# danikiyasseh/SAIS

Hardware: AMD Instinct MI355X
Metric: frames/sec ViT-S/16 fwd+bwd, 224x224 32-frame clips (higher is better)
Workload: dtype bf16; 1 GPU; BASELINE config 2: ViT-S/16 + 4-layer temporal encoder + SupCon prototype loss, fwd+bwd+SGD, 8 clips x 32 frames x 224x224 per GPU (global 8 clips), random-init weights, RGB stream; clips_per_gpu=8, frames_per_clip=32, streams=1, parallelism=dp1, launch=hipGraph replay, last_block_cls_only=True

## Files before the change

sais_amd/csrc/gemm.hip:

```cpp
#include "gemm_nt_tile.hpp"

namespace {

template <int EPI>
__global__ __launch_bounds__(256) void gemm_nt_kernel(NtParams p) {
    __shared__ __attribute__((aligned(16))) char smem[4 * TILE_BYTES];
    const int tid = threadIdx.x, lane = tid & 63;
    const int wid = __builtin_amdgcn_readfirstlane(tid >> 6);
    const int wr = wid >> 1, wc = wid & 1, g = lane >> 4, li = lane & 15;
    const int ntn = p.N / BN;
    const int tile = xcd_remap(blockIdx.x, gridDim.x);
    const int n0 = (tile % ntn) * BN, m0 = (tile / ntn) * BM;

    const int sub = lane >> 3, spos = lane & 7, schunk = spos ^ sub;
    const bf16* asrc[4]; const bf16* bsrc[4];
#pragma unroll
    for (int j = 0; j < 4; ++j) {
        const int r = 8 * (4 * wid + j) + sub;
        int m = m0 + r;
        m = m < p.M ? m : p.M - 1;
        asrc[j] = p.A + (size_t)m * p.lda + schunk * 8;
        bsrc[j] = p.B + (size_t)(n0 + perm_row(r)) * p.ldb + schunk * 8;
    }
    auto issue = [&](int stage, int k0) {
        char* s = smem + stage * 2 * TILE_BYTES + (4 * wid) * 1024;
#pragma unroll
        for (int j = 0; j < 4; ++j) {
            glds16(asrc[j] + k0, s + j * 1024);
            glds16(bsrc[j] + k0, s + TILE_BYTES + j * 1024);
        }
    };

    f32x4 acc[4][4];
#pragma unroll
    for (int i = 0; i < 4; ++i)
#pragma unroll
        for (int j = 0; j < 4; ++j) acc[i][j] = f32x4{0, 0, 0, 0};

    int nk = p.K / BK, kbase = 0;
    if constexpr (EPI == SAIS_EPI_RAW_SLABS_F32) {
        const int per = (nk + (int)gridDim.y - 1) / (int)gridDim.y;
        kbase = blockIdx.y * per;
        nk = min(per, nk - kbase);
        if (nk <= 0) nk = 0;
    }
    if (nk > 0) issue(0, kbase * BK);
    __syncthreads();
    float bias[16];
    EpiAux aux;
    for (int kt = 0; kt < nk; ++kt) {
        const int cur = kt & 1;
        if (kt + 1 < nk) issue(cur ^ 1, (kbase + kt + 1) * BK);
        const char* sa = smem + cur * 2 * TILE_BYTES;
        const char* sb = sa + TILE_BYTES;
        if constexpr (EPI != SAIS_EPI_RAW_SLABS_F32)
            if (kt == nk - 1) epilogue_loads<EPI>(p, m0 + wr * 64, li, n0 + wc * 64 + 16 * g, bias, aux);
#pragma unroll
        for (int ks = 0; ks < 2; ++ks) {
            bf16x8 fa[4], fb[4];
#pragma unroll
            for (int t = 0; t < 4; ++t) {
                fa[t] = *(const bf16x8*)(sa + swz(wr * 64 + t * 16 + li, ks * 4 + g));
                fb[t] = *(const bf16x8*)(sb + swz(wc * 64 + t * 16 + li, ks * 4 + g));
            }
#pragma unroll
            for (int mt = 0; mt < 4; ++mt)
#pragma unroll
                for (int nt = 0; nt < 4; ++nt) acc[mt][nt] = mfma16(fb[nt], fa[mt], acc[mt][nt]);
        }
        __syncthreads();
    }

#pragma unroll
    for (int mt = 0; mt < 4; ++mt) {
        int m = m0 + wr * 64 + mt * 16 + li;
        if (m >= p.M) continue;
        float v[16];
#pragma unroll
        for (int nt = 0; nt < 4; ++nt)
#pragma unroll
            for (int r = 0; r < 4; ++r) v[4 * nt + r] = acc[mt][nt][r];
        if constexpr (EPI == SAIS_EPI_RAW_SLABS_F32) {
            float* o = (float*)p.out + ((size_t)blockIdx.y * p.M + m) * p.ldo + n0 + wc * 64 + 16 * g;
#pragma unroll
            for (int i = 0; i < 4; ++i) *(f32x4*)(o + 4 * i) = f32x4{v[4 * i], v[4 * i + 1], v[4 * i + 2], v[4 * i + 3]};
        } else {
            epilogue<EPI>(p, m, n0 + wc * 64 + 16 * g, v, bias, aux, mt);
        }
    }
}

__global__ __launch_bounds__(256) void splitk_finish_kernel(const float* ws, int ks, int M, int N, int lds, const float* bias,
                                                            const float* rowscale, const float* aux, int ldaux, float* out32,
                                                            int ldo32, bf16* out16, int ldo16) {
    const int n4 = N >> 2;
    for (long i = blockIdx.x * 256L + threadIdx.x; i < (long)M * n4; i += (long)gridDim.x * 256) {
        const int m = (int)(i / n4), n = (int)(i - (long)m * n4) * 4;
        f32x4 y = *(const f32x4*)(ws + (size_t)m * lds + n);
        for (int z = 1; z < ks; ++z) y += *(const f32x4*)(ws + ((size_t)z * M + m) * lds + n);
        if (bias) y += *(const f32x4*)(bias + n);
        if (rowscale) y *= rowscale[m];
        if (aux) y += *(const f32x4*)(aux + (size_t)m * ldaux + n);
        if (out32) *(f32x4*)(out32 + (size_t)m * ldo32 + n) = y;
        if (out16) {
            bf16x4 o;
            o[0] = (bf16)y[0]; o[1] = (bf16)y[1]; o[2] = (bf16)y[2]; o[3] = (bf16)y[3];
            *(bf16x4*)(out16 + (size_t)m * ldo16 + n) = o;
        }
    }
}

#ifdef SAIS_NT_STAMP
__device__ unsigned long long g_nt_stamps[8][16];
#define NTSTAMP(i) do { if (blockIdx.x == 0 && titer == 2 && lane == 0) g_nt_stamps[wid][i] = __builtin_readcyclecounter(); } while (0)
#else
#define NTSTAMP(i) do { } while (0)
#endif
#ifndef SAIS_NT_ABL
#define SAIS_NT_ABL 0
#endif
template <int EPI>
__global__ __launch_bounds__(512, 2) void gemm_nt_w8p_kernel(NtParams p, int ntiles) {
    extern __shared__ __attribute__((aligned(16))) char smem[];
    CLK_STAMP(EPI == SAIS_EPI_BIAS_GELU_GRAD_BF16 ? 1 : EPI == SAIS_EPI_MUL_BF16 ? 2 : 0);
    [[maybe_unused]] const int abl_role = (SAIS_NT_ABL & 4) ? (blockIdx.x & 1) : (SAIS_NT_ABL & 8) ? ((blockIdx.x >> 8) & 1) : -1;
    const bool do_k = !(SAIS_NT_ABL & 1) && abl_role != 1, do_e = !(SAIS_NT_ABL & 2) && abl_role != 0;
    const int tid = threadIdx.x, lane = tid & 63;
    const int wid = __builtin_amdgcn_readfirstlane(tid >> 6);
    const int wr = wid >> 2, wc = wid & 3, g = lane >> 4, li = lane & 15;
    const int ntn = p.N / BN;
    const int sub = lane >> 3, spos = lane & 7, schunk = spos ^ sub;
    const bf16* asrc[2]; const bf16* bsrc[2];
    auto set_tile = [&](int v, int& m0, int& n0) {
        const int tile = xcd_remap(v, ntiles);
        n0 = (tile % ntn) * BN; m0 = (tile / ntn) * BM;
#pragma unroll
        for (int j = 0; j < 2; ++j) {
            const int r = 8 * (2 * wid + j) + sub;
            int m = m0 + r;
            m = m < p.M ? m : p.M - 1;
            asrc[j] = p.A + (size_t)m * p.lda + schunk * 8;
            bsrc[j] = p.B + (size_t)(n0 + perm_row32(r)) * p.ldb + schunk * 8;
        }
    };
    char* const sW = smem + 3 * TILE_BYTES;
    auto issue_a = [&](int kt) {
        char* s = smem + (kt % 3) * TILE_BYTES + (2 * wid) * 1024;
#pragma unroll
        for (int j = 0; j < 2; ++j) glds16(asrc[j] + kt * BK, s + j * 1024);
    };
    auto issue_w = [&](int kt) {
        char* s = sW + (kt & 1) * TILE_BYTES + (2 * wid) * 1024;
#pragma unroll
        for (int j = 0; j < 2; ++j) glds16(bsrc[j] + kt * BK, s + j * 1024);
    };
    const int nk = p.K / BK;
    constexpr int SROW = (EPI == SAIS_EPI_BIAS_F32) ? 2 : (EPI == SAIS_EPI_BIAS_RESID_F32) ? 2 : (EPI == SAIS_EPI_PATCH_F32) ? 2
                       : (EPI == SAIS_EPI_BIAS_GELU_GRAD_BF16 || EPI == SAIS_EPI_BIAS_GELU_GRADQ_BF16) ? 2 : 1;
    const int nstores = 4 * (SROW + ((EPI == SAIS_EPI_BIAS_RESID_F32 || EPI == SAIS_EPI_BIAS_GELU_BF16) && p.out2 ? 1 : 0));

    const bool do_pf = nk == 6 && ntn >= 8 && ntn <= 16 && wid == 0;
    unsigned pf_keep = 0;
    auto prefetch_a = [&](int pm0, int tcol) {
        const int per = (BM + ntn - 1) / ntn;
        const int row = tcol * per + (lane >> 2);
        if ((lane >> 2) < per && row < BM) {
            int m = pm0 + row;
            m = m < p.M ? m : p.M - 1;
            const bf16* q = p.A + (size_t)m * p.lda + (2 + (lane & 3)) * 64;
            asm volatile("global_load_dword %0, %1, off" : "=v"(pf_keep) : "v"(q) : "memory");
        }
    };
    int v = blockIdx.x, m0, n0;
    if (v >= ntiles) return;
    set_tile(v, m0, n0);
    if (do_k) {
        issue_a(0);
        issue_w(0);
        if (nk > 1) issue_a(1);
    }
    if (nk > 1) asm volatile("s_waitcnt vmcnt(2)" ::: "memory"); else asm volatile("s_waitcnt vmcnt(0)" ::: "memory");
    __builtin_amdgcn_s_barrier();
    [[maybe_unused]] int titer = -1;
    for (;;) {
        ++titer;
        NTSTAMP(0);
        f32x4 acc[4][2];
#pragma unroll
        for (int i = 0; i < 4; ++i)
#pragma unroll
            for (int j = 0; j < 2; ++j) acc[i][j] = f32x4{0, 0, 0, 0};
        float bias[8];
        EpiAux8 aux;
        __builtin_amdgcn_s_setprio(2);
        for (int kt = 0; kt < (do_k ? nk : 0); ++kt) {
            if (kt + 1 < nk) issue_w(kt + 1);
            if (kt + 2 < nk) issue_a(kt + 2);
            const char* sa = smem + (kt % 3) * TILE_BYTES;
            const char* sb = sW + (kt & 1) * TILE_BYTES;
            if (kt == nk - 1 && do_e) epilogue_loads8<EPI>(p, m0 + wr * 64, li, n0 + wc * 32 + 8 * g, bias, aux);
#pragma unroll
            for (int ks = 0; ks < 2; ++ks) {
                bf16x8 fa[4], fb[2];
#pragma unroll
                for (int t = 0; t < 4; ++t) fa[t] = *(const bf16x8*)(sa + swz(wr * 64 + t * 16 + li, ks * 4 + g));
#pragma unroll
                for (int t = 0; t < 2; ++t) fb[t] = *(const bf16x8*)(sb + swz(wc * 32 + t * 16 + li, ks * 4 + g));
#pragma unroll
                for (int mt = 0; mt < 4; ++mt)
#pragma unroll
                    for (int nt = 0; nt < 2; ++nt) acc[mt][nt] = mfma16(fb[nt], fa[mt], acc[mt][nt]);
            }
            if (kt + 2 < nk) asm volatile("s_waitcnt vmcnt(2) lgkmcnt(0)" ::: "memory");
            else if (kt + 1 < nk) asm volatile("s_waitcnt vmcnt(0) lgkmcnt(0)" ::: "memory");
            else asm volatile("s_waitcnt lgkmcnt(0)" ::: "memory");
            NTSTAMP(1 + 2 * kt);
            __builtin_amdgcn_s_barrier();
            NTSTAMP(2 + 2 * kt);
        }
        __builtin_amdgcn_s_setprio(0);
        const int cm0 = m0, cn0 = n0;
        const int nv = v + gridDim.x;
        const bool more = nv < ntiles;
        asm volatile("" ::"v"(pf_keep));
        if (more) {
            set_tile(nv, m0, n0);
            if (do_k) {
                issue_a(0);
                issue_w(0);
                if (nk > 1) issue_a(1);
                if (do_pf) prefetch_a(m0, xcd_remap(nv, ntiles) % ntn);
            }
        }
        if (SAIS_NT_ABL) {
            if (!do_k) epilogue_loads8<EPI>(p, cm0 + wr * 64, li, cn0 + wc * 32 + 8 * g, bias, aux);
            if (!do_e) {
#pragma unroll
                for (int mt = 0; mt < 4; ++mt)
#pragma unroll
                    for (int nt = 0; nt < 2; ++nt) asm volatile("" ::"v"(acc[mt][nt]));
            }
        }
#pragma unroll
        for (int mt = 0; mt < (do_e ? 4 : 0); ++mt) {
            const int m = cm0 + wr * 64 + mt * 16 + li;
            if (m >= p.M) continue;
            float vv[8];
#pragma unroll
            for (int nt = 0; nt < 2; ++nt)
#pragma unroll
                for (int r = 0; r < 4; ++r) vv[4 * nt + r] = acc[mt][nt][r];
            epilogue8<EPI>(p, m, cn0 + wc * 32 + 8 * g, vv, bias, aux, mt);
        }
        NTSTAMP(13);
        if (!more) break;
        v = nv;
        const int allow = (cm0 + BM <= p.M && nk > 1) ? nstores + 2 + (do_pf ? 1 : 0) : 0;
        if (allow == 6) asm volatile("s_waitcnt vmcnt(6)" ::: "memory");
        else if (allow == 7) asm volatile("s_waitcnt vmcnt(7)" ::: "memory");
        else if (allow == 10) asm volatile("s_waitcnt vmcnt(10)" ::: "memory");
        else if (allow == 11) asm volatile("s_waitcnt vmcnt(11)" ::: "memory");
        else if (allow == 14) asm volatile("s_waitcnt vmcnt(14)" ::: "memory");
        else if (allow == 15) asm volatile("s_waitcnt vmcnt(15)" ::: "memory");
        else asm volatile("s_waitcnt vmcnt(0)" ::: "memory");
        NTSTAMP(14);
        __builtin_amdgcn_s_barrier();
        NTSTAMP(15);
    }
}

#ifdef SAIS_NT_STAMP
extern "C" int sais_debug_nt_stamps(unsigned long long* host_out) {
    return hipMemcpyFromSymbol(host_out, HIP_SYMBOL(g_nt_stamps), sizeof(unsigned long long) * 8 * 16) == hipSuccess ? 0 : -2;
}
#endif

}

extern "C" int sais_gemm_nt_row_(const SaisGemm* g, void* stream);
extern "C" int sais_gemm_nt_exp_(const SaisGemm* g, int nt_grid, void* stream);
CLK_EXPORT(gemm)

template <int E>
static int launch_nt(const NtParams& p, dim3 grid, bool big, int nt_grid, hipStream_t stream) {
    if (big) {
        if (!sais_dyn_lds_once<gemm_nt_w8p_kernel<E>>(5 * TILE_BYTES)) return SAIS_ERR_LAUNCH;
        const int nt = (int)grid.x;
        hipLaunchKernelGGL(gemm_nt_w8p_kernel<E>, dim3(nt < nt_grid ? nt : nt_grid), dim3(512), 5 * TILE_BYTES, stream, p, nt);
    } else {
        hipLaunchKernelGGL(gemm_nt_kernel<E>, grid, dim3(256), 0, stream, p);
    }
    return sais_check_launch();
}
#define NT_CASE(E) case E: return launch_nt<E>(p, grid, big, nt_grid, (hipStream_t)stream);

extern "C" int sais_gemm_nt(const SaisGemm* g, void* stream) {
    SAIS_ENTER();
    if (!g || !g->A || !g->B || !g->out) return SAIS_ERR_ARG;
    if (g->M <= 0 || g->N % BN || g->K % BK || g->lda % 8 || g->ldb % 8 || g->ldo % 8) return SAIS_ERR_ARG;
    if ((g->epilogue == SAIS_EPI_BIAS_GELU_GRAD_BF16 || g->epilogue == SAIS_EPI_BIAS_GELU_GRADQ_BF16) && !g->out2) return SAIS_ERR_ARG;
    if (g->epilogue == SAIS_EPI_BIAS_GELU_GRADQ_BF16 && (g->ldo2 % 16 || ((uintptr_t)g->out2 & 15))) return SAIS_ERR_ARG;
    if (g->epilogue == SAIS_EPI_MULQ_BF16 && (!g->aux || g->ldaux % 16 || ((uintptr_t)g->aux & 15))) return SAIS_ERR_ARG;
    if ((g->epilogue == SAIS_EPI_MUL_BF16 || g->epilogue == SAIS_EPI_DGELU_BF16 || g->epilogue == SAIS_EPI_DRELU_BF16 ||
         g->epilogue == SAIS_EPI_BIAS_RESID_F32) && !g->aux)
        return SAIS_ERR_ARG;
    const NtParams p = nt_params(g);
    if (g->rowscale && g->epilogue != SAIS_EPI_BIAS_RESID_F32) return SAIS_ERR_ARG;
    const dim3 grid = nt_tiles(g);
    const bool big = g->M >= 8192;
    static const int nt_grid_env = sais_env_int("SAIS_NT_GRID", 0);
    const int nt_grid = nt_grid_env > 0 ? nt_grid_env : 512;
    if (g->epilogue == SAIS_EPI_RAW_SLABS_F32) {
        if (big || g->grp_in < 1 || g->grp_in > g->K / BK || g->ldo % 4) return SAIS_ERR_ARG;
        hipLaunchKernelGGL(gemm_nt_kernel<SAIS_EPI_RAW_SLABS_F32>, dim3(grid.x, g->grp_in), dim3(256), 0, (hipStream_t)stream, p);
        return sais_check_launch();
    }
    if (big && g->N == 384 && (g->epilogue == SAIS_EPI_BIAS_BF16 || (g->epilogue == SAIS_EPI_BIAS_RESID_F32 && !g->out2)))
        return sais_gemm_nt_row_(g, stream);
    if (big && g->rowscale) return SAIS_ERR_ARG;
#if SAIS_EXPERIMENTAL
    if (big)
        if (const int r = sais_gemm_nt_exp_(g, nt_grid, stream)) return r > 0 ? SAIS_OK : r;
#endif
    switch (g->epilogue) {
        NT_EPILOGUES(NT_CASE)
        default: return SAIS_ERR_ARG;
    }
#undef NT_CASE
}

extern "C" int sais_splitk_finish(const float* slabs, int nslabs, int M, int N, int lds, const float* bias,
                                  const float* rowscale, const float* aux, int ldaux, float* out32, int ldo32, void* out16,
                                  int ldo16, void* stream) {
    SAIS_ENTER();
    if (!slabs || nslabs < 1 || M <= 0 || N <= 0 || N % 4 || lds % 4 || (!out32 && !out16)) return SAIS_ERR_ARG;
    if ((aux && ldaux % 4) || (out32 && ldo32 % 4) || (out16 && ldo16 % 4)) return SAIS_ERR_ARG;
    const long n = (long)M * (N / 4);
    const int grid = (int)((n + 255) / 256 < 1024 ? (n + 255) / 256 : 1024);
    hipLaunchKernelGGL(splitk_finish_kernel, dim3(grid), dim3(256), 0, (hipStream_t)stream, slabs, nslabs, M, N, lds, bias,
                       rowscale, aux, ldaux, out32, ldo32, (bf16*)out16, ldo16);
    return sais_check_launch();
}
```

Measured before the change: 20870 frames/s.

## Add persistent 256x256 macro-tile NT GEMM kernel for large-M, K=384 shapes

Adds a persistent 1024-thread GEMM kernel with 256x256 output tiles for large-M NT GEMMs whose K equals six BK steps (K=384 for ViT-S). It triple-buffers A, double-buffers W in LDS, and overlaps the next tile's first loads with the current epilogue to cut per-tile global traffic and launch/tail overhead. It is routed ahead of the existing w8p path when the tile count is large enough. The larger tile means fewer waves per CU and heavier register use, and the kernel only applies to one K value.

```diff
diff --git a/sais_amd/csrc/gemm.hip b/sais_amd/csrc/gemm.hip
--- a/sais_amd/csrc/gemm.hip
+++ b/sais_amd/csrc/gemm.hip
@@ -279,6 +279,7 @@
 
 extern "C" int sais_gemm_nt_row_(const SaisGemm* g, void* stream);
 extern "C" int sais_gemm_nt_exp_(const SaisGemm* g, int nt_grid, void* stream);
+extern "C" int sais_gemm_nt_macro_(const SaisGemm* g, void* stream);
 CLK_EXPORT(gemm)
 
 template <int E>
@@ -322,6 +323,8 @@
     if (big)
         if (const int r = sais_gemm_nt_exp_(g, nt_grid, stream)) return r > 0 ? SAIS_OK : r;
 #endif
+    if (big)
+        if (const int r = sais_gemm_nt_macro_(g, stream)) return r > 0 ? SAIS_OK : r;
     switch (g->epilogue) {
         NT_EPILOGUES(NT_CASE)
         default: return SAIS_ERR_ARG;
diff --git a/sais_amd/csrc/gemm_nt_macro.hip b/sais_amd/csrc/gemm_nt_macro.hip
--- /dev/null
+++ b/sais_amd/csrc/gemm_nt_macro.hip
@@ -0,0 +1,229 @@
+#include "gemm_nt_tile.hpp"
+#include <type_traits>
+
+namespace {
+
+constexpr int MT = 256;
+constexpr int SLOT = MT * BK * 2;
+constexpr int NK = 6;
+constexpr int MACRO_LDS = 5 * SLOT;
+constexpr int MACRO_GRID = 256;
+
+template <int EPI>
+constexpr bool light_loads = !(EPI == SAIS_EPI_BIAS_RESID_F32 || EPI == SAIS_EPI_PATCH_F32 || EPI == SAIS_EPI_MUL_BF16 ||
+                               EPI == SAIS_EPI_DGELU_BF16 || EPI == SAIS_EPI_DRELU_BF16);
+
+template <int K> using Step = std::integral_constant<int, K>;
+
+DEVINL unsigned kbytes(unsigned b) {
+    asm volatile("" : "+s"(b));
+    return b;
+}
+
+DEVINL int fresh(int lane) {
+    asm volatile("" : "+v"(lane));
+    return lane;
+}
+
+DEVINL unsigned lds_addr(const void* p) { return (unsigned)(uintptr_t)(const __attribute__((address_space(3))) char*)p; }
+DEVINL bf16x8 lds_frag(unsigned addr) { return *(const bf16x8 __attribute__((address_space(3)))*)(uintptr_t)addr; }
+
+template <int EPI>
+DEVINL void settle_loads(float (&b)[8], EpiAux8& a) {
+#pragma unroll
+    for (int i = 0; i < 8; ++i) asm volatile("" : "+v"(b[i]));
+#pragma unroll
+    for (int mt = 0; mt < 4; ++mt) {
+        if constexpr (EPI == SAIS_EPI_BIAS_RESID_F32 || EPI == SAIS_EPI_PATCH_F32) {
+            asm volatile("" : "+v"(a.r[mt][0]), "+v"(a.r[mt][1]));
+        } else if constexpr (EPI == SAIS_EPI_DGELU_BF16 || EPI == SAIS_EPI_DRELU_BF16 || EPI == SAIS_EPI_MUL_BF16) {
+            u32x4 t = __builtin_bit_cast(u32x4, a.u[mt]);
+            asm volatile("" : "+v"(t));
+            a.u[mt] = __builtin_bit_cast(bf16x8, t);
+        } else if constexpr (EPI == SAIS_EPI_MULQ_BF16) {
+            asm volatile("" : "+v"(a.q[mt]));
+        }
+    }
+}
+
+template <int EPI>
+__global__ __launch_bounds__(1024) void gemm_nt_macro_kernel(NtParams p, int ntiles) {
+    extern __shared__ __attribute__((aligned(16))) char smem[];
+    const int tid = threadIdx.x, lane = tid & 63;
+    const int wid = __builtin_amdgcn_readfirstlane(tid >> 6);
+    const int wr = wid >> 2, wc = wid & 3;
+    const int ntn = p.N / MT;
+    unsigned asrc[2], bsrc;
+    auto set_tile = [&](int v, int& m0, int& n0) {
+        const int l = fresh(lane), sub = l >> 3, schunk = (l & 7) ^ sub;
+        const int tile = xcd_remap(v, ntiles);
+        n0 = (tile % ntn) * MT; m0 = (tile / ntn) * MT;
+#pragma unroll
+        for (int j = 0; j < 2; ++j) {
+            const int r = 8 * (2 * wid + j) + sub;
+            int m = m0 + r;
+            m = m < p.M ? m : p.M - 1;
+            asrc[j] = ((unsigned)m * p.lda + schunk * 8) * 2;
+        }
+        bsrc = ((unsigned)(n0 + perm_row32(16 * wid + sub)) * p.ldb + schunk * 8) * 2;
+    };
+    char* const sW = smem + 3 * SLOT;
+    auto issue_a = [&](auto KT) {
+        constexpr int kt = decltype(KT)::value;
+        char* s = smem + (kt % 3) * SLOT + (2 * wid) * 1024;
+#pragma unroll
+        for (int j = 0; j < 2; ++j) glds16((const char*)p.A + kbytes(kt * BK * 2) + asrc[j], s + j * 1024);
+    };
+    auto issue_w = [&](auto KT) {
+        constexpr int kt = decltype(KT)::value;
+        char* s = sW + (kt & 1) * SLOT + (2 * wid) * 1024;
+#pragma unroll
+        for (int j = 0; j < 2; ++j) glds16((const char*)p.B + (kbytes(kt * BK * 2) + (size_t)j * 32 * p.ldb) + bsrc, s + j * 1024);
+    };
+    auto first_loads = [&]() {
+        issue_a(Step<0>{});
+        issue_w(Step<0>{});
+        issue_a(Step<1>{});
+    };
+    constexpr int SROW = (EPI == SAIS_EPI_BIAS_F32) ? 2 : (EPI == SAIS_EPI_BIAS_RESID_F32) ? 2 : (EPI == SAIS_EPI_PATCH_F32) ? 2
+                       : (EPI == SAIS_EPI_BIAS_GELU_GRAD_BF16 || EPI == SAIS_EPI_BIAS_GELU_GRADQ_BF16) ? 2 : 1;
+    const int nstores = 4 * (SROW + ((EPI == SAIS_EPI_BIAS_RESID_F32 || EPI == SAIS_EPI_BIAS_GELU_BF16) && p.out2 ? 1 : 0));
+
+    const int pf_per = (MT + ntn - 1) / ntn;
+    const bool do_pf = light_loads<EPI> && EPI != SAIS_EPI_MULQ_BF16 && ntn >= 4 && wid * 16 < pf_per;
+    unsigned pf_keep = 0;
+    auto prefetch_a = [&](int pm0, int tcol) {
+        const int l = fresh(lane), own = wid * 16 + (l >> 2), row = tcol * pf_per + own;
+        if (own < pf_per && row < MT) {
+            int m = pm0 + row;
+            m = m < p.M ? m : p.M - 1;
+            const bf16* q = p.A + (size_t)m * p.lda + (2 + (l & 3)) * 64;
+            asm volatile("global_load_dword %0, %1, off" : "=v"(pf_keep) : "v"(q) : "memory");
+        }
+    };
+    int v = blockIdx.x, m0, n0;
+    if (v >= ntiles) return;
+    set_tile(v, m0, n0);
+    first_loads();
+    asm volatile("s_waitcnt vmcnt(2)" ::: "memory");
+    __builtin_amdgcn_s_barrier();
+    for (;;) {
+        const int fl = fresh(lane);
+        const unsigned frag0 = swz(fl & 15, fl >> 4);
+        const unsigned afrag = lds_addr(smem) + wr * 64 * 128, wfrag = lds_addr(sW) + wc * 64 * 128;
+        f32x4 acc[4][4];
+#pragma unroll
+        for (int i = 0; i < 4; ++i)
+#pragma unroll
+            for (int j = 0; j < 4; ++j) acc[i][j] = f32x4{0, 0, 0, 0};
+        float bias[2][8];
+        EpiAux8 aux[2];
+        __builtin_amdgcn_s_setprio(2);
+        auto kstep = [&](auto KT) {
+            constexpr int kt = decltype(KT)::value;
+            if constexpr (kt + 1 < NK) issue_w(Step<kt + 1>{});
+            if constexpr (kt + 2 < NK) issue_a(Step<kt + 2>{});
+            constexpr int aslot = (kt % 3) * SLOT, wslot = (kt & 1) * SLOT;
+#pragma unroll
+            for (int ks = 0; ks < 2; ++ks) {
+                bf16x8 fa[4], fb[4];
+                const unsigned fo = frag0 ^ (ks << 6);
+#pragma unroll
+                for (int t = 0; t < 4; ++t) fa[t] = lds_frag(afrag + fo + aslot + t * 2048);
+#pragma unroll
+                for (int t = 0; t < 4; ++t) fb[t] = lds_frag(wfrag + fo + wslot + t * 2048);
+#pragma unroll
+                for (int mt = 0; mt < 4; ++mt)
+#pragma unroll
+                    for (int nt = 0; nt < 4; ++nt) acc[mt][nt] = mfma16(fb[nt], fa[mt], acc[mt][nt]);
+                __builtin_amdgcn_sched_barrier(0);
+            }
+            if constexpr (kt == NK - 1 && light_loads<EPI>) {
+                __builtin_amdgcn_sched_barrier(0);
+                const int l = fresh(lane);
+#pragma unroll
+                for (int h = 0; h < 2; ++h)
+                    epilogue_loads8<EPI>(p, m0 + wr * 64, l & 15, n0 + wc * 64 + h * 32 + 8 * (l >> 4), bias[h], aux[h]);
+            }
+            if constexpr (kt + 2 < NK) asm volatile("s_waitcnt vmcnt(2) lgkmcnt(0)" ::: "memory");
+            else if constexpr (kt + 1 < NK) asm volatile("s_waitcnt vmcnt(0) lgkmcnt(0)" ::: "memory");
+            else asm volatile("s_waitcnt lgkmcnt(0)" ::: "memory");
+            __builtin_amdgcn_s_barrier();
+        };
+        kstep(Step<0>{}); kstep(Step<1>{}); kstep(Step<2>{}); kstep(Step<3>{}); kstep(Step<4>{}); kstep(Step<5>{});
+        __builtin_amdgcn_s_setprio(0);
+        const int cm0 = m0, cn0 = n0;
+        const int nv = v + gridDim.x;
+        const bool more = nv < ntiles;
+        asm volatile("" ::"v"(pf_keep));
+        if constexpr (light_loads<EPI>) {
+            settle_loads<EPI>(bias[0], aux[0]);
+            settle_loads<EPI>(bias[1], aux[1]);
+        }
+        auto next_tile = [&]() {
+            if (more) {
+                set_tile(nv, m0, n0);
+                first_loads();
+                if (do_pf) prefetch_a(m0, xcd_remap(nv, ntiles) % ntn);
+            }
+        };
+        if constexpr (light_loads<EPI>) next_tile();
+        const int el = fresh(lane), eg = el >> 4, eli = el & 15;
+#pragma unroll
+        for (int h = 0; h < 2; ++h) {
+            const int n = cn0 + wc * 64 + h * 32 + 8 * eg;
+            if constexpr (!light_loads<EPI>) {
+                epilogue_loads8<EPI>(p, cm0 + wr * 64, eli, n, bias[h], aux[h]);
+                settle_loads<EPI>(bias[h], aux[h]);
+            }
+#pragma unroll
+            for (int mt = 0; mt < 4; ++mt) {
+                const int m = cm0 + wr * 64 + mt * 16 + eli;
+                if (m >= p.M) continue;
+                float vv[8];
+#pragma unroll
+                for (int nt = 0; nt < 2; ++nt)
+#pragma unroll
+                    for (int r = 0; r < 4; ++r) vv[4 * nt + r] = acc[mt][2 * h + nt][r];
+                epilogue8<EPI>(p, m, n, vv, bias[h], aux[h], mt);
+            }
+        }
+        if constexpr (!light_loads<EPI>) next_tile();
+        if (!more) break;
+        v = nv;
+        const int allow = light_loads<EPI> && cm0 + MT <= p.M ? nstores : 0;
+        if (allow == 4) asm volatile("s_waitcnt vmcnt(4)" ::: "memory");
+        else if (allow == 8) asm volatile("s_waitcnt vmcnt(8)" ::: "memory");
+        else asm volatile("s_waitcnt vmcnt(0)" ::: "memory");
+        __builtin_amdgcn_s_barrier();
+    }
+}
+
+template <int E>
+int launch_macro(const NtParams& p, int tiles, hipStream_t stream) {
+    if (!sais_dyn_lds_once<gemm_nt_macro_kernel<E>>(MACRO_LDS)) return SAIS_ERR_LAUNCH;
+    hipLaunchKernelGGL(gemm_nt_macro_kernel<E>, dim3(tiles < MACRO_GRID ? tiles : MACRO_GRID), dim3(1024), MACRO_LDS, stream, p,
+                       tiles);
+    return sais_check_launch();
+}
+
+}
+
+extern "C" int sais_gemm_nt_macro_rule_(int M, int N, int K, int mode) {
+    if (mode <= 0 || K != NK * BK || N <= 0 || N % MT || M < 8192) return 0;
+    const long tiles = (long)((M + MT - 1) / MT) * (N / MT);
+    return mode >= 2 || tiles >= 4 * MACRO_GRID;
+}
+
+extern "C" int sais_gemm_nt_macro_(const SaisGemm* g, void* stream) {
+    if (!sais_gemm_nt_macro_rule_(g->M, g->N, g->K, sais_env_int("SAIS_NT_MACRO", 1))) return 0;
+    if ((uint64_t)g->M * g->lda * 2 >= (1ull << 32) || (uint64_t)g->N * g->ldb * 2 >= (1ull << 32) || g->lda < 0 || g->ldb < 0) return 0;
+    const NtParams p = nt_params(g);
+    const int tiles = ((g->M + MT - 1) / MT) * (g->N / MT);
+#define MACRO_CASE(E) case E: { const int r = launch_macro<E>(p, tiles, (hipStream_t)stream); return r == SAIS_OK ? 1 : r; }
+    switch (g->epilogue) {
+        NT_EPILOGUES(MACRO_CASE)
+        default: return 0;
+    }
+#undef MACRO_CASE
+}
```

New measurement: 21020 frames/s (median of 6 runs). No clear change (+0.7%).
